# pmgbergen/porepy

Hardware: NVIDIA H100
Metric: 3D cells/sec MPFA+MPSA assembly (higher is better)
Workload: dtype f64

## Files before the change

porepy_b200/csrc/api.cu:

```cuda
#include <cuda_runtime.h>

#include <omp.h>

#include <atomic>
#include <chrono>
#include <thread>
#include <climits>
#include <cstdio>
#include <cstdlib>
#include <cstring>
#include <string>
#include <vector>

#include "plan.hpp"
#include <nvtx3/nvToolsExt.h>

struct NvtxRange {
    explicit NvtxRange(const char *name) { nvtxRangePushA(name); }
    ~NvtxRange() { nvtxRangePop(); }
};

static thread_local std::string g_err;
static thread_local int64_t g_err_node = -1;
static std::atomic<int64_t> g_launches{0};
// ... 27 lines not shown
void pb_set_error_node_(int64_t node) { g_err_node = node; }
extern "C" int64_t pb_launch_count(void) { return g_launches.load(); }
extern "C" int pb_device_count(void) {
    int n = 0;
    if (cudaGetDeviceCount(&n) != cudaSuccess) return -1;
    return n;
}
extern "C" int pb_set_device(int device) {
    CUDA_TRY(cudaSetDevice(device));
    return PB_OK;
}

extern "C" int pb_host_alloc(uint64_t bytes, void **out) {
    if (!out) return fail(PB_EINVAL, "null pointer");
    CUDA_TRY(cudaHostAlloc(out, bytes ? bytes : 8, cudaHostAllocDefault));
    return PB_OK;
}
extern "C" void pb_host_free(void *p) {
    if (p) cudaFreeHost(p);
}

static int64_t cfg_scratch(int cfg, int n) {
    switch (cfg) {
        case 0: return Cfg0::scratch_doubles_c();
        case 1: return Cfg1::scratch_doubles_c();
        case 2: return Cfg2::scratch_doubles_c();
        case 3: return Cfg3::scratch_doubles_c();
        case 4: return Cfg4::scratch_doubles_c();
        case 5: return Cfg5::scratch_doubles_c();
        default: return n;
    }
}

template <class F>
static int build_classes(pb_plan *p, std::vector<NodeClass> &out, F size_of) {
    const HostPlan &H = p->H;
    std::vector<int32_t> lists[2 * kNumCfg];
    int64_t amax[2 * kNumCfg] = {0}, rmax[2 * kNumCfg] = {0}, smax[2 * kNumCfg] = {0};
    for (int64_t s = 0; s < H.nn; ++s) {
        int nsc = H.node_sc_ptr[s + 1] - H.node_sc_ptr[s];
        int nsf = H.node_sf_ptr[s + 1] - H.node_sf_ptr[s];
        if (nsf == 0) continue;
        if (!p->active.empty() && !p->active[s]) continue;
        int n = 0, w = 0;
        int64_t a = 0, r = 0;
        size_of(nsf, nsc, H.node_nb[s], &n, &w, &a, &r);
        int cfg = 0;
        while (cfg < kCatchAll && (n > kCfg[cfg].max_n || w > kCfg[cfg].max_w)) ++cfg;
        const int64_t scr = cfg_scratch(cfg, n);
        const int tpb = kCfg[cfg].team == 32 ? 4 : 1;
        bool glob = (size_t)(a + r + scr) * 8 * tpb > kMaxSmem;
        if (glob && (size_t)(r + scr) * 8 * tpb > kMaxSmem)
            return fail(PB_ENOTIMPL, "interaction region at node " + std::to_string(s) +
                                         " is too large for this build (" + std::to_string(nsf) +
                                         " sub-faces)");
        int key = cfg * 2 + (glob ? 1 : 0);
        lists[key].push_back((int32_t)s);
        amax[key] = std::max(amax[key], a);
        rmax[key] = std::max(rmax[key], r);
        smax[key] = std::max(smax[key], scr);
    }
    out.clear();
    for (int key = 0; key < 2 * kNumCfg; ++key) {
        if (lists[key].empty()) continue;
        out.emplace_back();
        NodeClass &c = out.back();
        c.cfg = key / 2;
        c.a_global = key & 1;
        c.team = kCfg[c.cfg].team;
        c.n = (int)lists[key].size();
        c.a_doubles = amax[key];
        c.rest_doubles = rmax[key];
        c.scr_doubles = smax[key];
        if (!c.a_global) {
            const int tpb = c.team == 32 ? 4 : 1;
            if ((size_t)(c.a_doubles + c.rest_doubles + c.scr_doubles) * 8 * tpb > kMaxSmem) c.a_global = true;
        }
        if (!p->node_key.empty()) {
            const std::vector<uint32_t> &nk = p->node_key;
            std::stable_sort(lists[key].begin(), lists[key].end(), [&](int32_t x, int32_t y) { return nk[x] < nk[y]; });
        }
        if (c.nodes.upload(lists[key], p->stream) != cudaSuccess) return fail(PB_ECUDA, "upload of node list failed");
    }
    return PB_OK;
}

static int build_mpfa_classes(pb_plan *p) {
    const int nd = p->H.nd;
    return build_classes(p, p->mpfa_cls, [&](int nsf, int nsc, int nb, int *n, int *w, int64_t *a, int64_t *r) {
        *n = nsf;
        *w = mpfa_width(nd, nsf, nsc, nb);
        *a = mpfa_A_doubles(nd, nsf, nsc, nb);
        *r = mpfa_rest_doubles(nd, nsf, nsc, nb);
    });
}

template <int CAP>
__global__ void pattern_kernel(int64_t nrows, const int32_t *__restrict__ rn_ptr, const int32_t *__restrict__ rn,
                               const int32_t *__restrict__ col_ptr, const int32_t *__restrict__ col_idx,
                               int32_t *__restrict__ counts, const int32_t *__restrict__ indptr,
                               int32_t *__restrict__ indices, int pass, int *overflow) {
    __shared__ int32_t sbuf[8][CAP];
    const int lane = threadIdx.x & 31, wib = threadIdx.x >> 5;
    int32_t *buf = sbuf[wib];
    const int64_t warp = (int64_t)blockIdx.x * (blockDim.x >> 5) + wib;
    const int64_t nwarps = (int64_t)gridDim.x * (blockDim.x >> 5);
    for (int64_t r = warp; r < nrows; r += nwarps) {
        int total = 0;
        bool over = false;
        for (int q = rn_ptr[r]; q < rn_ptr[r + 1]; ++q) {
            const int s = rn[q];
            const int b = col_ptr[s], len = col_ptr[s + 1] - b;
            if (total + len > CAP) { over = true; break; }
            for (int i = lane; i < len; i += 32) buf[total + i] = col_idx[b + i];
            total += len;
        }
        if (over) {
            if (lane == 0) { atomicExch(overflow, 1); if (pass == 0) counts[r] = 0; }
            continue;
        }
        int P = 1;
        while (P < total) P <<= 1;
// ... 951 lines not shown
    return PB_OK;
}

extern "C" int pb_mpsa_upload(pb_plan *p, const double *stiffness, const uint8_t *bc,
                              const double *robin_weight, double eta, int n_alpha,
                              const double *alpha) {
    NvtxRange nvtx_("pb_mpsa_upload");
    if (!p || !stiffness || !bc) return fail(PB_EINVAL, "null pointer");
    if (!p->have_geo) return fail(PB_EINVAL, "pb_plan_set_geometry has not been called");
    if (n_alpha < 0 || n_alpha > PB_MAX_ALPHA) return fail(PB_EINVAL, "0 <= n_alpha <= 4");
    if (n_alpha > 0 && !alpha) return fail(PB_EINVAL, "null alpha");
    const HostPlan &H = p->H;
    const int nd = H.nd;
    cudaStream_t st = p->stream;
    { int rcs = upload_cell_tensor(p, p->stiff, stiffness, 81); if (rcs) return rcs; }
    CUDA_TRY(p->vbc.upload(bc, (size_t)nd * H.nf, st));
    p->have_vrobw = robin_weight != nullptr;
    p->have_vbasis = false;
    if (robin_weight) CUDA_TRY(p->vrobw.upload(robin_weight, (size_t)nd * nd * H.nf, st));
    if (n_alpha) {
        CUDA_TRY(p->alpha.ensure((size_t)n_alpha * 9 * H.nc * sizeof(double)));
        for (int q = 0; q < n_alpha; ++q) {
            DevBuf one;
            int rca = upload_cell_tensor(p, one, alpha + (size_t)q * 9 * (p->cell_map.p ? p->cell_map_src : H.nc), 9);
            if (rca) return rca;
            CUDA_TRY(cudaMemcpyAsync(p->alpha.as<double>() + (size_t)q * 9 * H.nc, one.p,
                                     (size_t)9 * H.nc * sizeof(double), cudaMemcpyDeviceToDevice, st));
            CUDA_TRY(cudaStreamSynchronize(st));
        }
    }
    p->n_alpha = n_alpha;
    p->veta = eta;
    if (p->mpsa_cls_nalpha != n_alpha) {
        int rc = build_classes(p, p->mpsa_cls, [&](int nsf, int nsc, int nb, int *n, int *w, int64_t *a,
                                                   int64_t *r) {
            *n = nsf * nd;
            *w = mpsa_width(nd, nsf, nsc, nb, n_alpha);
            *a = mpsa_A_doubles(nd, nsf, nsc, nb, n_alpha);
            *r = mpsa_rest_doubles(nd, nsf, nsc, nb, n_alpha);
        });
        if (rc) return rc;
        p->mpsa_cls_nalpha = n_alpha;
    }
    CUDA_TRY(cudaStreamSynchronize(st));
    p->mpsa_ready = true;
    return PB_OK;
}

extern "C" int pb_mpsa_set_basis(pb_plan *p, const double *basis) {
    if (!p) return fail(PB_EINVAL, "null plan");
    if (!p->mpsa_ready) return fail(PB_EINVAL, "pb_mpsa_upload has not been called");
    p->have_vbasis = basis != nullptr;
    if (basis) {
        const HostPlan &H = p->H;
        CUDA_TRY(p->vbasis.upload(basis, (size_t)H.nd * H.nd * H.nf, p->stream));
        CUDA_TRY(cudaStreamSynchronize(p->stream));
    }
    return PB_OK;
}

extern "C" int pb_mpsa_assemble(pb_plan *p, float *ms) {
    NvtxRange nvtx_("pb_mpsa_assemble");
    if (!p) return fail(PB_EINVAL, "null plan");
    if (!p->mpsa_ready) return fail(PB_EINVAL, "pb_mpsa_upload has not been called");
    const HostPlan &H = p->H;
    const int nd = H.nd;
    cudaStream_t st = p->stream;
    const size_t nfc = (size_t)p->pat_nnz[0], nfb = (size_t)p->pat_nnz[1], ncc = (size_t)p->pat_nnz[2], ncb = (size_t)p->pat_nnz[3];
// ... 63 lines not shown
```

porepy_b200/csrc/mpsa_node.cuh:

```cuda
#pragma once
#include "node_kernels.cuh"

namespace pb {

PB_HD int mpsa_width(int nd, int nsf, int nsc, int nb, int nalpha) {
    return (nsf * nd + nsc * nd + nb * nd + nalpha * nsc) | 1;
}
PB_HD int64_t mpsa_A_doubles(int nd, int nsf, int nsc, int nb, int nalpha) {
    return (int64_t)nsf * nd * mpsa_width(nd, nsf, nsc, nb, nalpha);
}
PB_HD int64_t mpsa_rest_doubles(int nd, int nsf, int nsc, int nb, int nalpha) {
    const int64_t nd2 = nd * nd, n = (int64_t)nsf * nd;
    const int64_t nrhs = (int64_t)nsc * nd + (int64_t)nb * nd + (int64_t)nalpha * nsc;
    int64_t d = (int64_t)nsc * nd2 * nd2;
    d += (int64_t)nsc * nd2;
    d += nd2 * (n + (int64_t)nsc * nd);
    d += nd2 * nrhs;
    d += nsf;
    d += (int64_t)nsf * nd;
    d += (int64_t)nsc;
    d += (int64_t)nalpha * nsc * nd2 * 2;
    int64_t ints = nsc + 4 * (int64_t)nsf + (int64_t)nsf * nd + n + (int64_t)nsc * nd + 2 * nd;
    return d + (ints + 1) / 2 + 2;
}

template <int ND>
PB_HD int c9(int i, int r) { return 3 * i + r; }

template <int ND>
PB_HD bool sym_mask(int p, int q) {
    if (p == q) return true;
    return (p % (ND + 1) == 0) && (q % (ND + 1) == 0);
}

template <int ND, class Solver, class Team>
PB_HD void mpsa_node(Team &t, const PlanView &P, const GeoView &G, const MpsaParams &prm,
                     const MpsaOut &o, int64_t s, double *A, double *smd, double *scratch, int *err,
                     int64_t s_next = -1) {
    constexpr int ND2 = ND * ND;
    const int sc0 = P.node_sc_ptr[s], nsc = P.node_sc_ptr[s + 1] - sc0;
    const int sf0 = P.node_sf_ptr[s], nsf = P.node_sf_ptr[s + 1] - sf0;
    const int nb = P.node_nb[s];
    if (nsf == 0) return;
    const int nal = prm.n_alpha;
    const int n = nsf * ND;
    const int ncc = nsc * ND;
    const int nbc = nb * ND;
    const int nrhs = ncc + nbc + nal * nsc;
    const int W = (n + nrhs) | 1;
    const int64_t nf = P.nf, nc = P.nc, nn = P.nn;

    double *PS = smd;
    double *E = PS + nsc * ND2 * ND2;
    double *SA = E + nsc * ND2;
    double *SAc = SA + ND2 * n;
    double *Z = SAc + ND2 * ncc;
    double *invmf = Z + ND2 * nrhs;
    double *nrm = invmf + nsf;
    double *volk = nrm + nsf * ND;
    double *NA = volk + nsc;
    double *AE = NA + nal * nsc * ND2;
    int *cell = (int *)(AE + nal * nsc * ND2);
    int *face = cell + nsc;
    int *sides = face + nsf;
    int *bloc = sides + nsf;
    int *bcu = bloc + nsf;
    int *rowidx = bcu + nsf * ND;
    int *slot = rowidx + n;
    int *elim = slot + nsc * ND;
    int *sidesel = elim + 2 * ND;

    for (int k = t.tid(); k < nsc; k += t.size()) cell[k] = P.sc_cell[sc0 + k];
    for (int i = t.tid(); i < nsc * ND; i += t.size()) slot[i] = P.slot_sf[(int64_t)sc0 * ND + i];
    for (int u = t.tid(); u < nsf; u += t.size()) {
        const int64_t f = P.sf_face[sf0 + u];
        face[u] = (int)f;
        sides[u] = (int)P.sf_sides[sf0 + u];
        const int bl = P.sf_bloc[sf0 + u];
        bloc[u] = (bl == 0xFFFF) ? -1 : bl;
        const double im = 1.0 / (double)(P.fn_indptr[f + 1] - P.fn_indptr[f]);
        invmf[u] = im;
#pragma unroll
        for (int i = 0; i < ND; ++i) {
            int code = 0;
            if (bl != 0xFFFF) {
                code = prm.bc[i * nf + f];
                if (code == 0) code = 2;
            }
            bcu[u * ND + i] = code;
            nrm[u * ND + i] = G.fnorm[i * G.face_cs + f * G.face_es] * im;
        }
    }
    for (int x = t.tid(); x < n; x += t.size()) rowidx[x] = x;
    for (int i = t.tid(); i < n * W; i += t.size()) A[i] = 0.0;
    for (int i = t.tid(); i < ND2 * (n + ncc); i += t.size()) SA[i] = 0.0;
    t.sync();

    for (int k = t.tid(); k < nsc; k += t.size()) {
        const int64_t c = cell[k];
        double xc[ND], xs[ND], D[ND][ND], Ei[ND][ND];
#pragma unroll
        for (int i = 0; i < ND; ++i) {
            xc[i] = G.ccent[i * G.cell_cs + c * G.cell_es];
            xs[i] = G.nodes[i * G.node_cs + s * G.node_es];
        }
#pragma unroll
        for (int m = 0; m < ND; ++m) {
            const int u = slot[k * ND + m] >> 1;
            const int64_t f = face[u];
            const double e = (bloc[u] >= 0) ? 0.0 : prm.eta;
#pragma unroll
            for (int i = 0; i < ND; ++i) {
                const double xf = G.fcent[i * G.face_cs + f * G.face_es];
                D[m][i] = xf + e * (xs[i] - xf) - xc[i];
            }
        }
        if (!invert_small<ND>(D, Ei)) flag_singular(err, s);
#pragma unroll
        for (int q = 0; q < ND; ++q)
#pragma unroll
            for (int m = 0; m < ND; ++m) E[k * ND2 + q * ND + m] = Ei[q][m];
        volk[k] = G.cvol[c] / (double)P.sc_ncn[c];
        for (int q = 0; q < nal; ++q) {
            const double *al = prm.alpha + (int64_t)q * prm.alpha_stride;
            double a2[ND][ND];
#pragma unroll
            for (int a = 0; a < ND; ++a)
// ... 66 lines not shown
        for (int u = 0; u < nsf; ++u) {
            cn += bcu[u * ND + i] == 2;
            cr += bcu[u * ND + i] == 3;
        }
        elim[i] = nsc < cn;
        elim[ND + i] = nsc < cr;
    }
    t.sync();

    for (int u = t.tid(); u < nsf; u += t.size()) {
        const int s1 = sides[u] & 0xFFFF, s2 = (sides[u] >> 16) & 0xFFFF;
        int pick = s1;
        if (s2 != 0xFFFF) {
            const double *nu = nrm + u * ND;
            double w1 = 0.0, w2 = 0.0;
            const double *p1 = PS + (s1 / ND) * ND2 * ND2, *p2 = PS + (s2 / ND) * ND2 * ND2;
            for (int i = 0; i < ND; ++i)
                for (int am = 0; am < ND2; ++am) {
                    double a1 = 0.0, a2 = 0.0;
#pragma unroll
                    for (int r = 0; r < ND; ++r) {
                        a1 += nu[r] * p1[(i * ND + r) * ND2 + am];
                        a2 += nu[r] * p2[(i * ND + r) * ND2 + am];
                    }
                    w1 += fabs(a1);
                    w2 += fabs(a2);
                }
            if (w2 < w1) pick = s2;
        }
        sidesel[u] = pick;
    }
    t.sync();

    for (int x = t.tid(); x < n; x += t.size()) {
        const int u = x / ND, i = x - u * ND;
        double *row = A + (int64_t)x * W;
        const int code = bcu[x];
        if (code == 1 && prm.basis == nullptr) {
            row[x] = 1.0;
            row[n + ncc + bloc[u] * ND + i] = 1.0;
            continue;
        }
        const double *nu = nrm + u * ND;
        if (prm.basis != nullptr && bloc[u] >= 0) {
            const int64_t fb = face[u];
            double B[ND][ND];
#pragma unroll
            for (int a = 0; a < ND; ++a)
#pragma unroll
                for (int j = 0; j < ND; ++j) B[a][j] = prm.basis[(int64_t)(a * ND + j) * nf + fb];
            if (code == 1) {
#pragma unroll
                for (int j = 0; j < ND; ++j) row[u * ND + j] = B[i][j];
                row[n + ncc + bloc[u] * ND + i] = 1.0;
            } else {
                const int side = sides[u] & 0xFFFF;
                const int k = side / ND;
                const double sg = (slot[side] & 1) ? -1.0 : 1.0;
                for (int j = 0; j < ND; ++j) {
                    const double wgt = sg * B[i][j];
                    if (wgt == 0.0) continue;
                    const double *ps = PS + (k * ND2 + j * ND) * ND2;
#pragma unroll
                    for (int a = 0; a < ND; ++a) {
                        double csum = 0.0;
#pragma unroll
                        for (int m = 0; m < ND; ++m) {
                            double v = 0.0;
#pragma unroll
                            for (int r = 0; r < ND; ++r) v += nu[r] * ps[(r * ND + a) * ND + m];
                            v *= wgt;
                            row[(slot[k * ND + m] >> 1) * ND + a] += v;
                            csum += v;
                        }
                        row[n + k * ND + a] += csum;
                    }
                    for (int q = 0; q < nal; ++q)
                        row[n + ncc + nbc + q * nsc + k] += wgt * NA[((q * nsc + k) * ND + (side - k * ND)) * ND + j];
                    const int cj = bcu[u * ND + j];
                    if (!((cj == 2 && elim[j]) || (cj == 3 && elim[ND + j]))) {
                        for (int c = 0; c < n; ++c) {
                            double v = 0.0;
#pragma unroll
                            for (int r = 0; r < ND; ++r) v += nu[r] * SA[(j * ND + r) * n + c];
                            row[c] += wgt * v;
                        }
                        for (int c = 0; c < ncc; ++c) {
                            double v = 0.0;
#pragma unroll
                            for (int r = 0; r < ND; ++r) v += nu[r] * SAc[(j * ND + r) * ncc + c];
                            row[n + c] -= wgt * v;
                        }
                    }
                }
                row[n + ncc + bloc[u] * ND + i] = invmf[u];
                if (code == 3) {
                    const double as = G.farea[fb] * invmf[u];
#pragma unroll
                    for (int j = 0; j < ND; ++j) {
                        double wb = 0.0;
#pragma unroll
                        for (int kk = 0; kk < ND; ++kk)
                            wb += (prm.robw ? prm.robw[(int64_t)(i * ND + kk) * nf + fb] : (i == kk ? 1.0 : 0.0)) * B[kk][j];
                        row[u * ND + j] += as * wb;
                    }
                }
            }
            double sum = 0.0;
            for (int c = 0; c < n; ++c) sum += fabs(row[c]);
            if (!(sum > 0.0)) { flag_singular(err, s); continue; }
            const double is = 1.0 / sum;
            for (int c = 0; c < n + nrhs; ++c) row[c] *= is;
            continue;
        }
        for (int sd = 0; sd < 2; ++sd) {
            const int side = sd == 0 ? (sides[u] & 0xFFFF) : ((sides[u] >> 16) & 0xFFFF);
            if (side == 0xFFFF) continue;
            const int k = side / ND;
            const double sg = (slot[side] & 1) ? -1.0 : 1.0;
            const double *ps = PS + (k * ND2 + i * ND) * ND2;
#pragma unroll
            for (int a = 0; a < ND; ++a) {
                double csum = 0.0;
#pragma unroll
                for (int m = 0; m < ND; ++m) {
                    double v = 0.0;
#pragma unroll
                    for (int r = 0; r < ND; ++r) v += nu[r] * ps[(r * ND + a) * ND + m];
                    v *= sg;
                    row[(slot[k * ND + m] >> 1) * ND + a] += v;
                    csum += v;
                }
                row[n + k * ND + a] += csum;
            }
            for (int q = 0; q < nal; ++q)
                row[n + ncc + nbc + q * nsc + k] += sg * NA[((q * nsc + k) * ND + (side - k * ND)) * ND + i];
            if (code != 0) {
                const bool el = code == 2 ? elim[i] : elim[ND + i];
                if (!el) {
                    for (int c = 0; c < n; ++c) {
                        double v = 0.0;
#pragma unroll
                        for (int r = 0; r < ND; ++r) v += nu[r] * SA[(i * ND + r) * n + c];
                        row[c] += sg * v;
                    }
                    for (int c = 0; c < ncc; ++c) {
                        double v = 0.0;
#pragma unroll
                        for (int r = 0; r < ND; ++r) v += nu[r] * SAc[(i * ND + r) * ncc + c];
                        row[n + c] -= sg * v;
                    }
                }
            }
        }
        if (code == 2 || code == 3) row[n + ncc + bloc[u] * ND + i] = invmf[u];
        if (code == 3) {
            const int64_t f = face[u];
            const double as = G.farea[f] * invmf[u];
#pragma unroll
            for (int j = 0; j < ND; ++j) {
                const double w = prm.robw ? prm.robw[(int64_t)(i * ND + j) * nf + f] : (i == j ? 1.0 : 0.0);
                row[u * ND + j] += as * w;
            }
        }
        double sum = 0.0;
        for (int c = 0; c < n; ++c) sum += fabs(row[c]);
        if (!(sum > 0.0)) { flag_singular(err, s); continue; }
        const double is = 1.0 / sum;
        for (int c = 0; c < n + nrhs; ++c) row[c] *= is;
    }
    t.sync();

    if (!Solver::solve(t, A, n, W, nrhs, rowidx, scratch)) {
        if (t.tid() == 0) flag_singular(err, s);
        t.sync();
        return;
    }

#if defined(__CUDA_ARCH__)
    int pf_sc0 = 0, pf_nsc = 0, pf_sf0 = 0, pf_nsf = 0;
    int64_t pf_pos0 = 0;
    if (s_next >= 0) {
        pf_sc0 = P.node_sc_ptr[s_next];
        pf_nsc = P.node_sc_ptr[s_next + 1] - pf_sc0;
        pf_sf0 = P.node_sf_ptr[s_next];
        pf_nsf = P.node_sf_ptr[s_next + 1] - pf_sf0;
        pf_pos0 = P.posfc_ptr[s_next];
    }
#endif
#if defined(__CUDA_ARCH__)
    {
        const int l = t.lane();
        const int ntr = (ND2 + 15) / 16, ntc = (nrhs + 7) / 8;
        for (int tile = t.warp(); tile < ntr * ntc; tile += t.nwarps()) {
            const int tr = tile / ntc, tc = tile - tr * ntc;
            const int row0 = 16 * tr + (l >> 2), row1 = row0 + 8;
            const int colb = 8 * tc + (l >> 2);
            double acc0[2] = {0.0, 0.0}, acc1[2] = {0.0, 0.0};
            for (int k0 = 0; k0 < n; k0 += 4) {
                const int k = k0 + (l & 3);
                const double a0 = (row0 < ND2 && k < n) ? SA[row0 * n + k] : 0.0;
                const double a1 = (row1 < ND2 && k < n) ? SA[row1 * n + k] : 0.0;
                const double b = (k < n && colb < nrhs) ? A[(int64_t)rowidx[k] * W + n + colb] : 0.0;
                pb_dmma2(acc0, acc1, a0, a1, b);
            }
            const int c0 = 8 * tc + 2 * (l & 3);
            const int rows[2] = {row0, row1};
            const double *accs[2] = {acc0, acc1};
            for (int h = 0; h < 2; ++h) {
                const int row = rows[h];
                if (row < ND2) {
                    if (c0 < nrhs) Z[row * nrhs + c0] = accs[h][0] + (c0 < ncc ? SAc[row * ncc + c0] : 0.0);
                    if (c0 + 1 < nrhs)
                        Z[row * nrhs + c0 + 1] = accs[h][1] + (c0 + 1 < ncc ? SAc[row * ncc + c0 + 1] : 0.0);
                }
            }
        }
    }
#else
    for (int it = t.tid(); it < ND2 * nrhs; it += t.size()) {
        const int p = it / nrhs, c = it - p * nrhs;
        double v = (c < ncc) ? SAc[p * ncc + c] : 0.0;
        for (int x = 0; x < n; ++x) v += SA[p * n + x] * A[(int64_t)rowidx[x] * W + n + c];
        Z[it] = v;
    }
#endif
    t.sync();

#if defined(__CUDA_ARCH__)
    int pf_cell = -1, pf_face = -1;
    if (t.tid() < pf_nsc) pf_cell = P.sc_cell[pf_sc0 + t.tid()];
    if (t.tid() < pf_nsf) {
        pf_face = P.sf_face[pf_sf0 + t.tid()];
        if ((t.tid() & 7) == 0) {
            pb_prefetch_l2(P.sf_sides + pf_sf0 + t.tid());
            pb_prefetch_l2(P.sf_bloc + pf_sf0 + t.tid());
        }
    }
    if (t.tid() * 16 < pf_nsc * ND) pb_prefetch_l2(P.slot_sf + (int64_t)pf_sc0 * ND + t.tid() * 16);
    for (int64_t off = (int64_t)t.tid() * 32; off < (int64_t)pf_nsf * pf_nsc; off += (int64_t)t.size() * 32)
        pb_prefetch_l2(P.pos_fc + pf_pos0 + off);
#endif
    const int32_t *pfc = P.pos_fc + P.posfc_ptr[s];
    const int32_t *pfb = P.pos_fb + P.posfb_ptr[s];
    for (int u = t.warp(); u < nsf; u += t.nwarps()) {
        const double *nu = nrm + u * ND;
        const int side1 = sidesel[u];
        const int k1 = side1 / ND, m1 = side1 - k1 * ND;
        double hs[ND][ND][ND];
        double hsum[ND][ND];
#pragma unroll
        for (int i = 0; i < ND; ++i) {
            const double *ps1 = PS + (k1 * ND2 + i * ND) * ND2;
#pragma unroll
            for (int a = 0; a < ND; ++a) {
                double sm = 0.0;
#pragma unroll
                for (int m = 0; m < ND; ++m) {
                    double v = 0.0;
#pragma unroll
                    for (int r = 0; r < ND; ++r) v += nu[r] * ps1[(r * ND + a) * ND + m];
                    hs[i][a][m] = v;
                    sm += v;
                }
                hsum[i][a] = sm;
            }
        }
        int xo[ND][ND];
#pragma unroll
        for (int a = 0; a < ND; ++a)
#pragma unroll
            for (int m = 0; m < ND; ++m) xo[a][m] = rowidx[(slot[k1 * ND + m] >> 1) * ND + a] * W + n;
        bool use_asym[ND];
        int uo[ND];
#pragma unroll
        for (int i = 0; i < ND; ++i) {
            const int code = bcu[u * ND + i];
            use_asym[i] = !((code == 2 && elim[i]) || (code == 3 && elim[ND + i]));
            uo[i] = rowidx[u * ND + i] * W + n;
        }
        const double im = invmf[u];
        const int64_t f = face[u];
        const int64_t fc0 = P.fc_indptr[f], fcl = P.fc_indptr[f + 1] - fc0;
        const int64_t fb0 = P.fb_indptr[f], fbl = P.fb_indptr[f + 1] - fb0;
        for (int c = t.lane(); c < nrhs; c += t.lanes()) {
            double hk[ND], tr[ND];
#pragma unroll
            for (int i = 0; i < ND; ++i) hk[i] = 0.0;
#pragma unroll
            for (int a = 0; a < ND; ++a)
#pragma unroll
                for (int m = 0; m < ND; ++m) {
                    const double xv = A[xo[a][m] + c];
#pragma unroll
                    for (int i = 0; i < ND; ++i) hk[i] += hs[i][a][m] * xv;
                }
#pragma unroll
            for (int i = 0; i < ND; ++i) {
                if (use_asym[i]) {
#pragma unroll
                    for (int r = 0; r < ND; ++r) hk[i] += nu[r] * Z[(i * ND + r) * nrhs + c];
                }
                tr[i] = A[uo[i] + c] * im;
            }
            if (c < ncc) {
                const int k = c / ND, j = c - k * ND;
                if (k == k1) {
#pragma unroll
                    for (int i = 0; i < ND; ++i) {
                        double hj = hsum[i][0];
#pragma unroll
                        for (int a = 1; a < ND; ++a) hj = (j == a) ? hsum[i][a] : hj;
                        hk[i] -= hj;
                    }
                }
                const int64_t pb = pfc[u * nsc + k];
                const int64_t pos = ND2 * fc0 + (pb - fc0) * ND + j;
#pragma unroll
                for (int i = 0; i < ND; ++i) {
                    if (o.stress) red_add(o.stress + pos + (int64_t)i * ND * fcl, hk[i]);
                    if (o.bdc) red_add(o.bdc + pos + (int64_t)i * ND * fcl, tr[i]);
                }
            } else if (c < ncc + nbc) {
                const int cb = c - ncc;
                const int b = cb / ND, j = cb - b * ND;
                const int64_t pb = pfb[u * nb + b];
                const int64_t pos = ND2 * fb0 + (pb - fb0) * ND + j;
#pragma unroll
                for (int i = 0; i < ND; ++i) {
                    if (o.bstress) red_add(o.bstress + pos + (int64_t)i * ND * fbl, hk[i]);
                    if (o.bdf) red_add(o.bdf + pos + (int64_t)i * ND * fbl, tr[i]);
                }
            } else {
                const int cq = c - ncc - nbc;
                const int q = cq / nsc, k = cq - q * nsc;
                const int64_t pb = pfc[u * nsc + k];
// ... 13 lines not shown
        if (prm.stiff_cs == 1) {
            const double *rec = prm.stiff + (int64_t)pf_cell * prm.stiff_es;
#pragma unroll
            for (int b = 0; b < 81; b += 16) pb_prefetch_l2(rec + b);
            pb_prefetch_l2(rec + 80);
        }
        if (G.cell_cs == 1) pb_prefetch_l2(G.ccent + (int64_t)pf_cell * G.cell_es);
        pb_prefetch_l2(G.cvol + pf_cell);
        pb_prefetch_l2(P.sc_ncn + pf_cell);
    }
    if (pf_face >= 0) {
        if (G.face_cs == 1) {
            pb_prefetch_l2(G.fnorm + (int64_t)pf_face * G.face_es);
            pb_prefetch_l2(G.fcent + (int64_t)pf_face * G.face_es);
        }
        pb_prefetch_l2(P.fn_indptr + pf_face);
        pb_prefetch_l2(P.fc_indptr + pf_face);
#pragma unroll
        for (int i = 0; i < ND; ++i) pb_prefetch_l2(prm.bc + (int64_t)i * nf + pf_face);
    }
#endif
    if (nal > 0) {
        const int32_t *pcc = P.pos_cc + P.poscc_ptr[s];
        const int32_t *pcb = P.pos_cb + P.poscb_ptr[s];
        for (int it = t.warp(); it < nal * nsc; it += t.nwarps()) {
            const int q = it / nsc, k = it - q * nsc;
            const double *ae = AE + (q * nsc + k) * ND2;
            const double vol = volk[k];
            const double *xr[ND][ND];
#pragma unroll
            for (int a = 0; a < ND; ++a)
#pragma unroll
                for (int m = 0; m < ND; ++m)
                    xr[a][m] = A + (int64_t)rowidx[(slot[k * ND + m] >> 1) * ND + a] * W + n;
            for (int c = t.lane(); c < nrhs; c += t.lanes()) {
                double v = 0.0;
#pragma unroll
                for (int a = 0; a < ND; ++a)
#pragma unroll
                    for (int m = 0; m < ND; ++m) v += ae[a * ND + m] * xr[a][m][c];
                if (c < ncc) {
                    const int k2 = c / ND, j = c - k2 * ND;
                    if (k2 == k) {
#pragma unroll
                        for (int m = 0; m < ND; ++m) v -= ae[j * ND + m];
                    }
                    if (o.dd[q]) red_add(o.dd[q] + (int64_t)pcc[k * nsc + k2] * ND + j, vol * v);
                } else if (c < ncc + nbc) {
                    const int cb = c - ncc;
                    const int b = cb / ND, j = cb - b * ND;
                    if (o.bdd[q]) red_add(o.bdd[q] + (int64_t)pcb[k * nb + b] * ND + j, vol * v);
                } else {
                    const int cq = c - ncc - nbc;
                    const int q2 = cq / nsc, k2 = cq - q2 * nsc;
                    if (q2 == q && o.cons[q]) red_add(o.cons[q] + (int64_t)pcc[k * nsc + k2], vol * v);
                }
            }
        }
    }
    t.sync();
}

}
```

porepy_b200/csrc/node_kernels.cuh:

```cuda
#pragma once
#include <cmath>
#include <cstdint>

#include "views.hpp"

namespace pb {

struct CpuTeam {
    PB_HD int tid() const { return 0; }
    PB_HD int size() const { return 1; }
    PB_HD int lanes() const { return 1; }
    PB_HD int warp() const { return 0; }
    PB_HD int nwarps() const { return 1; }
    PB_HD int lane() const { return 0; }
    PB_HD void sync() const {}
    PB_HD void warp_argmax(double &, int &) const {}
};

#if defined(__CUDACC__)
template <int TEAM>
struct GpuTeam {
    __device__ __forceinline__ int tid() const { return TEAM == 32 ? (threadIdx.x & 31) : threadIdx.x; }
    __device__ __forceinline__ int size() const { return TEAM; }
    __device__ __forceinline__ int lanes() const { return 32; }
// ... 51 lines not shown
            }
            t.warp_argmax(best, bi);
            if (t.lane() == 0) {
                int r = rowidx[bi];
                rowidx[bi] = rowidx[p];
                rowidx[p] = r;
                ipiv[p] = (best > 0.0) ? 1.0 / A[r * W + p] : 0.0;
            }
        }
        t.sync();
        const int pr = rowidx[p];
        const double inv = ipiv[p];
        if (inv == 0.0 || !(inv == inv)) ok = false;
        const int c0 = p + 1;
        const int wend = n + nrhs;
        for (int li = t.warp(); li < n; li += t.nwarps()) {
            if (li == p) continue;
            const int ri = rowidx[li];
            const double f = A[ri * W + p] * inv;
            if (f == 0.0) continue;
            for (int c = c0 + t.lane(); c < wend; c += t.lanes()) A[ri * W + c] -= f * A[pr * W + c];
        }
        t.sync();
    }
    for (int p = t.warp(); p < n; p += t.nwarps()) {
        const int pr = rowidx[p];
        const double inv = ipiv[p];
        for (int c = n + t.lane(); c < n + nrhs; c += t.lanes()) A[pr * W + c] *= inv;
    }
    t.sync();
    return ok;
}

struct SmemGJ {
    static constexpr int team = 256;
    static constexpr int min_blocks = 1;
    static PB_HD int64_t scratch_doubles(int n) { return n; }
    template <class Team>
    static PB_HD bool solve(Team &t, double *A, int n, int W, int nrhs, int *rowidx, double *scratch) {
        return gauss_jordan(t, A, n, W, nrhs, rowidx, scratch);
    }
};

#if defined(__CUDACC__)
__device__ __forceinline__ void pb_dmma(double (&c)[2], double a, double b) {
    asm volatile("mma.sync.aligned.m8n8k4.row.col.f64.f64.f64.f64 {%0,%1}, {%2}, {%3}, {%0,%1};"
                 : "+d"(c[0]), "+d"(c[1])
                 : "d"(a), "d"(b));
}
__device__ __forceinline__ void pb_dmma2(double (&c0)[2], double (&c1)[2], double a0, double a1, double b) {
    asm volatile("mma.sync.aligned.m16n8k4.row.col.f64.f64.f64.f64 {%0,%1,%2,%3}, {%4,%5}, {%6}, {%0,%1,%2,%3};"
                 : "+d"(c0[0]), "+d"(c0[1]), "+d"(c1[0]), "+d"(c1[1])
                 : "d"(a0), "d"(a1), "d"(b));
}

template <int NW, int RT, int NCT, int MINB>
struct TileGJ {
    static_assert(NCT % 2 == 0, "padded row stride must be 4 mod 16");
    static constexpr int team = NW * 32;
    static constexpr int min_blocks = MINB;
    static constexpr int NRT = NW * RT;
    static constexpr int max_n = NRT * 8;
    static constexpr int max_w = NCT * 8;
    static constexpr int NP = ((max_n + 31) / 32) * 32;
    static constexpr int NI = NP / 32;
    static constexpr int WP = NCT * 8 + 4;
    static_assert(NP <= 256, "row index must fit the 8-bit key field");
    static_assert(NI <= 8, "extend the PB_PICK list");
    static __host__ __device__ constexpr int64_t scratch_doubles_c() {
        return NP * 4 + 2 * 4 * WP + 16 * (NW + 1) + (8 + NP) / 2 + 4;
    }
    static PB_HD int64_t scratch_doubles(int) { return scratch_doubles_c(); }

// ... 95 lines not shown
                    const double rpiv = __drcp_rn(prow[j]);
#pragma unroll
                    for (int i = 0; i < NI; ++i) {
                        const bool me = (l == ol) && (i == os);
                        if (me) us[i] = true;
                        else {
                            const double f = v[i][j] * rpiv;
#pragma unroll
                            for (int jj = j + 1; jj < 4; ++jj) v[i][jj] -= f * prow[jj];
                        }
                    }
                }
            }
        }
        int prj = -1;
#pragma unroll
        for (int j = 0; j < 4; ++j)
            if (j == mj) prj = mypr[j];
        const double m = (prj >= 0) ? ((mi < pw) ? P0[prj * 4 + mi] : 0.0) : (mi == mj ? 1.0 : 0.0);
        const double growth = invert_block(l, m, iv);
        if (!(growth < 1e300)) sing = true;
        if (l < 16) Ainv[l] = iv;
        if (l == 0) {
#pragma unroll
            for (int j = 0; j < 4; ++j) {
                prs[j] = mypr[j];
                if (mypr[j] >= 0) { usedf[mypr[j]] = 1; rowidx[p0 + j] = mypr[j]; }
            }
            if (sing) prs[4] = 1;
        }
    }


    template <class Team>
    static __device__ __forceinline__ bool solve(Team &t, double *A, int n, int W, int nrhs,
                                                 int *rowidx, double *scratch) {
        const int ti = t.warp(), l = t.lane();
        const int gr = l >> 2, gc = (l & 3) * 2;
        const int wend = n + nrhs;
        double c[RT][NCT][2];
#pragma unroll
        for (int rt = 0; rt < RT; ++rt) {
            const int myrow = 8 * (ti + NW * rt) + gr;
#pragma unroll
            for (int tc = 0; tc < NCT; ++tc) {
                const int col = 8 * tc + gc;
                c[rt][tc][0] = (myrow < n && col < wend) ? A[myrow * W + col] : 0.0;
                c[rt][tc][1] = (myrow < n && col + 1 < wend) ? A[myrow * W + col + 1] : 0.0;
            }
        }
        double *P0 = scratch;
        double *Raw = P0 + NP * 4;
        double *R = Raw + 4 * WP;
        double *Ainv = R + 4 * WP;
        int *prs = (int *)(Ainv + 16 * (NW + 1));
        int *usedf = prs + 8;
        for (int i = t.tid(); i < NP; i += t.size()) usedf[i] = i < n ? 0 : 1;
        for (int i = t.tid(); i < NP * 4; i += t.size()) P0[i] = 0.0;
        if (t.tid() == 0) prs[4] = 0;
        t.sync();
        const int npanel = (n + 3) >> 2;
        bool ok = true;
#pragma unroll
        for (int tcp = 0; tcp < NRT && tcp < NCT; ++tcp) {
            for (int half = 0; half < 2; ++half) {
                const int q = 2 * tcp + half;
                if (q >= npanel || !ok) break;
                const int p0 = 4 * q;
                const int pw = (n - p0) < 4 ? (n - p0) : 4;
                if (((l & 3) >> 1) == half) {
                    const int j0 = 2 * (l & 1);
#pragma unroll
                    for (int rt = 0; rt < RT; ++rt) {
                        const int myrow = 8 * (ti + NW * rt) + gr;
                        P0[myrow * 4 + j0] = c[rt][tcp][0];
                        P0[myrow * 4 + j0 + 1] = c[rt][tcp][1];
                    }
                }
                int myp[RT];
#pragma unroll
                for (int rt = 0; rt < RT; ++rt) {
                    const int myrow = 8 * (ti + NW * rt) + gr;
                    const int j = myrow - p0;
// ... 56 lines not shown
                    rowidx[p0 + t.tid()] = p0 + t.tid();
                }
                {
                    const int k = l & 3;
                    const int src = (l & ~3) | (2 * half + (k >> 1));
                    double af[RT];
#pragma unroll
                    for (int rt = 0; rt < RT; ++rt) {
                        const double v0 = __shfl_sync(0xffffffffu, c[rt][tcp][0], src);
                        const double v1 = __shfl_sync(0xffffffffu, c[rt][tcp][1], src);
                        af[rt] = (k < pw) ? -((k & 1) ? v1 : v0) : 0.0;
                    }
                    const double *rb = R + k * WP + (l >> 2);
#pragma unroll
                    for (int tc = tcp; tc < NCT; ++tc) {
                        const double bf = rb[8 * tc];
#pragma unroll
                        for (int rt = 0; rt + 1 < RT; rt += 2) pb_dmma2(c[rt][tc], c[rt + 1][tc], af[rt], af[rt + 1], bf);
                        if (RT & 1) pb_dmma(c[RT - 1][tc], af[RT - 1], bf);
                    }
#pragma unroll
                    for (int rt = 0; rt < RT; ++rt)
                        if (myp[rt] >= 0) {
#pragma unroll
                            for (int tc = tcp; tc < NCT; ++tc) {
                                c[rt][tc][0] = R[myp[rt] * WP + 8 * tc + gc];
                                c[rt][tc][1] = R[myp[rt] * WP + 8 * tc + gc + 1];
                            }
                        }
                }
            }
        }
        t.sync();
        if (!ok) return false;
#pragma unroll
        for (int rt = 0; rt < RT; ++rt) {
            const int myrow = 8 * (ti + NW * rt) + gr;
#pragma unroll
            for (int tc = 0; tc < NCT; ++tc) {
                const int col = 8 * tc + gc;
                if (myrow < n) {
                    if (col >= n && col < wend) A[myrow * W + col] = c[rt][tc][0];
                    if (col + 1 >= n && col + 1 < wend) A[myrow * W + col + 1] = c[rt][tc][1];
                }
            }
        }
        t.sync();
        return true;
    }
};
#endif

#if defined(__CUDACC__)
__device__ __forceinline__ void pb_prefetch_l2(const void *p) {
    asm volatile("prefetch.global.L2 [%0];" ::"l"(p));
}
#endif

template <int ND>
PB_HD bool invert_small(const double (&D)[ND][ND], double (&E)[ND][ND]);

template <>
PB_HD bool invert_small<2>(const double (&D)[2][2], double (&E)[2][2]) {
    double det = D[0][0] * D[1][1] - D[0][1] * D[1][0];
    if (det == 0.0 || !(det == det)) return false;
    double id = 1.0 / det;
    E[0][0] = D[1][1] * id; E[0][1] = -D[0][1] * id;
    E[1][0] = -D[1][0] * id; E[1][1] = D[0][0] * id;
    return true;
}

template <>
PB_HD bool invert_small<3>(const double (&D)[3][3], double (&E)[3][3]) {
    double c00 = D[1][1] * D[2][2] - D[1][2] * D[2][1];
    double c01 = D[1][2] * D[2][0] - D[1][0] * D[2][2];
    double c02 = D[1][0] * D[2][1] - D[1][1] * D[2][0];
    double det = D[0][0] * c00 + D[0][1] * c01 + D[0][2] * c02;
    if (det == 0.0 || !(det == det)) return false;
    double id = 1.0 / det;
    E[0][0] = c00 * id;
    E[1][0] = c01 * id;
// ... 207 lines not shown
```

porepy_b200/csrc/plan.hpp:

```cpp
#pragma once
#include <cuda_runtime.h>

#include <algorithm>
#include <atomic>
#include <chrono>
#include <climits>
#include <cstdint>
#include <cstdio>
#include <cstdlib>
#include <cstring>
#include <map>
#include <mutex>
#include <string>
#include <vector>

#include "../../include/poreb200.h"
#include "mpsa_node.cuh"
#include "face_kernels.cuh"
#include "node_kernels.cuh"
#include "plan_host.hpp"

int pb_fail_(int code, const std::string &msg);
void pb_count_launch_();
void pb_set_error_node_(int64_t node);
// ... 162 lines not shown
    static int cache[64] = {0};
    int dev = 0;
    if (cudaGetDevice(&dev) != cudaSuccess || dev < 0 || dev >= 64) dev = 0;
    if (!cache[dev]) {
        int n = 0;
        if (cudaDeviceGetAttribute(&n, cudaDevAttrMultiProcessorCount, dev) != cudaSuccess || n < 1) n = 1;
        cache[dev] = n;
    }
    return cache[dev];
}


#define PB_LAUNCH_CFG(KERNEL, ND, ...)                                              \
    switch (c.cfg) {                                                                \
        case 0: rc = launch_one(KERNEL<ND, Cfg0>, c, p, __VA_ARGS__); break;        \
        case 1: rc = launch_one(KERNEL<ND, Cfg1>, c, p, __VA_ARGS__); break;        \
        case 2: rc = launch_one(KERNEL<ND, Cfg2>, c, p, __VA_ARGS__); break;        \
        case 3: rc = launch_one(KERNEL<ND, Cfg3>, c, p, __VA_ARGS__); break;        \
        case 4: rc = launch_one(KERNEL<ND, Cfg4>, c, p, __VA_ARGS__); break;        \
        case 5: rc = launch_one(KERNEL<ND, Cfg5>, c, p, __VA_ARGS__); break;        \
        default: rc = launch_one(KERNEL<ND, Cfg6>, c, p, __VA_ARGS__); break;       \
    }

template <class K, class Prm, class Out>
static int launch_one(K kernel, const NodeClass &c, pb_plan *p, const Prm &prm, const Out &o) {
    const int blk = c.team == 32 ? 128 : c.team;
    const int tpb = blk / c.team;
    const size_t smem = (size_t)(c.scr_doubles + c.rest_doubles + (c.a_global ? 0 : c.a_doubles)) *
                        sizeof(double) * tpb;
    if (smem > kMaxSmem)
        return pb_fail_(PB_ENOTIMPL, "interaction region needs " + std::to_string(smem) +
                                     " B of shared memory (> 227 KB)");
    CUDA_TRY(cudaFuncSetAttribute(kernel, cudaFuncAttributeMaxDynamicSharedMemorySize, (int)smem));
    int per_sm = 1;
    CUDA_TRY(cudaOccupancyMaxActiveBlocksPerMultiprocessor(&per_sm, kernel, blk, smem));
    if (per_sm < 1) per_sm = 1;
    int64_t need = ((int64_t)c.n + tpb - 1) / tpb;
    int grid = (int)std::max<int64_t>(1, std::min<int64_t>(need, (int64_t)pb_sm_count() * per_sm));
    double *ws = nullptr;
    if (c.a_global) {
        CUDA_TRY(p->a_ws.ensure((size_t)grid * tpb * c.a_doubles * sizeof(double)));
        ws = p->a_ws.as<double>();
    }
    kernel<<<grid, blk, smem, p->stream>>>(p->view, p->geo, prm, o, c.nodes.as<int32_t>(), c.n,
                                           (int)c.scr_doubles, (int)c.rest_doubles,
                                           (int)c.a_doubles, ws, p->err.as<int>());
    pb_count_launch_();
    CUDA_TRY(cudaGetLastError());
    return PB_OK;
}


int pb_launch_mpfa_(pb_plan *p, const MpfaParams &prm, const MpfaOut &o);
int pb_launch_mpsa2_(pb_plan *p, const MpsaParams &prm, const MpsaOut &o);
int pb_launch_mpsa3_(pb_plan *p, const MpsaParams &prm, const MpsaOut &o);
int pb_upload_repacked_(cudaStream_t st, DevBuf &tmp, DevBuf &dst, const double *host, int ncomp, int64_t n);
int pb_build_device_topology_(pb_plan *p, int nd, int64_t nc, int64_t nf, int64_t nn, const int32_t *cf_indptr,
                              const int32_t *cf_indices, const int8_t *cf_data, const int32_t *fn_indptr,
                              const int32_t *fn_indices, DevBuf &fn_idx_dev, std::string &err);
```

Before: 6.840 million.

## Fill MPSA rows directly into solver register tiles and shrink smem pool

MPSA assembly no longer builds the full n×W augmented matrix in shared memory. It passes a row-fill callback to the solver, which fills 8-row tiles per warp into a small buffer, normalises them and loads them straight into the elimination registers. The solution is then written to a compact padded X array. This reduces the per-node shared-memory footprint, which can raise occupancy or keep more nodes off the global-A path. A separate change sets the shared-memory carveout preference from the computed need, which may leave more L1 cache available.

```diff
diff --git a/porepy_b200/csrc/api.cu b/porepy_b200/csrc/api.cu
--- a/porepy_b200/csrc/api.cu
+++ b/porepy_b200/csrc/api.cu
@@ -83,8 +83,20 @@
     }
 }
 
+static int64_t cfg_pool(int cfg, int n, int w) {
+    switch (cfg) {
+        case 0: return Cfg0::pool_doubles(n, w);
+        case 1: return Cfg1::pool_doubles(n, w);
+        case 2: return Cfg2::pool_doubles(n, w);
+        case 3: return Cfg3::pool_doubles(n, w);
+        case 4: return Cfg4::pool_doubles(n, w);
+        case 5: return Cfg5::pool_doubles(n, w);
+        default: return Cfg6::pool_doubles(n, w);
+    }
+}
+
 template <class F>
-static int build_classes(pb_plan *p, std::vector<NodeClass> &out, F size_of) {
+static int build_classes(pb_plan *p, std::vector<NodeClass> &out, bool rows_to_solver, F size_of) {
     const HostPlan &H = p->H;
     std::vector<int32_t> lists[2 * kNumCfg];
     int64_t amax[2 * kNumCfg] = {0}, rmax[2 * kNumCfg] = {0}, smax[2 * kNumCfg] = {0};
@@ -107,7 +119,7 @@
                                          " sub-faces)");
         int key = cfg * 2 + (glob ? 1 : 0);
         lists[key].push_back((int32_t)s);
-        amax[key] = std::max(amax[key], a);
+        amax[key] = std::max(amax[key], rows_to_solver ? cfg_pool(cfg, n, w) : a);
         rmax[key] = std::max(rmax[key], r);
         smax[key] = std::max(smax[key], scr);
     }
@@ -138,7 +150,7 @@
 
 static int build_mpfa_classes(pb_plan *p) {
     const int nd = p->H.nd;
-    return build_classes(p, p->mpfa_cls, [&](int nsf, int nsc, int nb, int *n, int *w, int64_t *a, int64_t *r) {
+    return build_classes(p, p->mpfa_cls, false, [&](int nsf, int nsc, int nb, int *n, int *w, int64_t *a, int64_t *r) {
         *n = nsf;
         *w = mpfa_width(nd, nsf, nsc, nb);
         *a = mpfa_A_doubles(nd, nsf, nsc, nb);
@@ -1156,8 +1168,8 @@
     p->n_alpha = n_alpha;
     p->veta = eta;
     if (p->mpsa_cls_nalpha != n_alpha) {
-        int rc = build_classes(p, p->mpsa_cls, [&](int nsf, int nsc, int nb, int *n, int *w, int64_t *a,
-                                                   int64_t *r) {
+        int rc = build_classes(p, p->mpsa_cls, true, [&](int nsf, int nsc, int nb, int *n, int *w, int64_t *a,
+                                                         int64_t *r) {
             *n = nsf * nd;
             *w = mpsa_width(nd, nsf, nsc, nb, n_alpha);
             *a = mpsa_A_doubles(nd, nsf, nsc, nb, n_alpha);
diff --git a/porepy_b200/csrc/mpsa_node.cuh b/porepy_b200/csrc/mpsa_node.cuh
--- a/porepy_b200/csrc/mpsa_node.cuh
+++ b/porepy_b200/csrc/mpsa_node.cuh
@@ -35,7 +35,7 @@
 
 template <int ND, class Solver, class Team>
 PB_HD void mpsa_node(Team &t, const PlanView &P, const GeoView &G, const MpsaParams &prm,
-                     const MpsaOut &o, int64_t s, double *A, double *smd, double *scratch, int *err,
+                     const MpsaOut &o, int64_t s, double *pool, double *smd, double *scratch, int *err,
                      int64_t s_next = -1) {
     constexpr int ND2 = ND * ND;
     const int sc0 = P.node_sc_ptr[s], nsc = P.node_sc_ptr[s + 1] - sc0;
@@ -47,7 +47,6 @@
     const int ncc = nsc * ND;
     const int nbc = nb * ND;
     const int nrhs = ncc + nbc + nal * nsc;
-    const int W = (n + nrhs) | 1;
     const int64_t nf = P.nf, nc = P.nc, nn = P.nn;
 
     double *PS = smd;
@@ -92,7 +91,6 @@
         }
     }
     for (int x = t.tid(); x < n; x += t.size()) rowidx[x] = x;
-    for (int i = t.tid(); i < n * W; i += t.size()) A[i] = 0.0;
     for (int i = t.tid(); i < ND2 * (n + ncc); i += t.size()) SA[i] = 0.0;
     t.sync();
 
@@ -225,14 +223,13 @@
     }
     t.sync();
 
-    for (int x = t.tid(); x < n; x += t.size()) {
+    auto row_of = [&](int x, double *row) {
         const int u = x / ND, i = x - u * ND;
-        double *row = A + (int64_t)x * W;
         const int code = bcu[x];
         if (code == 1 && prm.basis == nullptr) {
             row[x] = 1.0;
             row[n + ncc + bloc[u] * ND + i] = 1.0;
-            continue;
+            return;
         }
         const double *nu = nrm + u * ND;
         if (prm.basis != nullptr && bloc[u] >= 0) {
@@ -299,12 +296,7 @@
                     }
                 }
             }
-            double sum = 0.0;
-            for (int c = 0; c < n; ++c) sum += fabs(row[c]);
-            if (!(sum > 0.0)) { flag_singular(err, s); continue; }
-            const double is = 1.0 / sum;
-            for (int c = 0; c < n + nrhs; ++c) row[c] *= is;
-            continue;
+            return;
         }
         for (int sd = 0; sd < 2; ++sd) {
             const int side = sd == 0 ? (sides[u] & 0xFFFF) : ((sides[u] >> 16) & 0xFFFF);
@@ -356,15 +348,11 @@
                 row[u * ND + j] += as * w;
             }
         }
-        double sum = 0.0;
-        for (int c = 0; c < n; ++c) sum += fabs(row[c]);
-        if (!(sum > 0.0)) { flag_singular(err, s); continue; }
-        const double is = 1.0 / sum;
-        for (int c = 0; c < n + nrhs; ++c) row[c] *= is;
-    }
-    t.sync();
-
-    if (!Solver::solve(t, A, n, W, nrhs, rowidx, scratch)) {
+    };
+
+    const double *X;
+    int ldx;
+    if (!Solver::solve_rows(t, row_of, n, nrhs, pool, rowidx, scratch, X, ldx)) {
         if (t.tid() == 0) flag_singular(err, s);
         t.sync();
         return;
@@ -394,7 +382,7 @@
                 const int k = k0 + (l & 3);
                 const double a0 = (row0 < ND2 && k < n) ? SA[row0 * n + k] : 0.0;
                 const double a1 = (row1 < ND2 && k < n) ? SA[row1 * n + k] : 0.0;
-                const double b = (k < n && colb < nrhs) ? A[(int64_t)rowidx[k] * W + n + colb] : 0.0;
+                const double b = (k < n && colb < nrhs) ? X[rowidx[k] * ldx + colb] : 0.0;
                 pb_dmma2(acc0, acc1, a0, a1, b);
             }
             const int c0 = 8 * tc + 2 * (l & 3);
@@ -414,7 +402,7 @@
     for (int it = t.tid(); it < ND2 * nrhs; it += t.size()) {
         const int p = it / nrhs, c = it - p * nrhs;
         double v = (c < ncc) ? SAc[p * ncc + c] : 0.0;
-        for (int x = 0; x < n; ++x) v += SA[p * n + x] * A[(int64_t)rowidx[x] * W + n + c];
+        for (int x = 0; x < n; ++x) v += SA[p * n + x] * X[(int64_t)rowidx[x] * ldx + c];
         Z[it] = v;
     }
 #endif
@@ -463,14 +451,14 @@
 #pragma unroll
         for (int a = 0; a < ND; ++a)
 #pragma unroll
-            for (int m = 0; m < ND; ++m) xo[a][m] = rowidx[(slot[k1 * ND + m] >> 1) * ND + a] * W + n;
+            for (int m = 0; m < ND; ++m) xo[a][m] = rowidx[(slot[k1 * ND + m] >> 1) * ND + a] * ldx;
         bool use_asym[ND];
         int uo[ND];
 #pragma unroll
         for (int i = 0; i < ND; ++i) {
             const int code = bcu[u * ND + i];
             use_asym[i] = !((code == 2 && elim[i]) || (code == 3 && elim[ND + i]));
-            uo[i] = rowidx[u * ND + i] * W + n;
+            uo[i] = rowidx[u * ND + i] * ldx;
         }
         const double im = invmf[u];
         const int64_t f = face[u];
@@ -484,7 +472,7 @@
             for (int a = 0; a < ND; ++a)
 #pragma unroll
                 for (int m = 0; m < ND; ++m) {
-                    const double xv = A[xo[a][m] + c];
+                    const double xv = X[xo[a][m] + c];
 #pragma unroll
                     for (int i = 0; i < ND; ++i) hk[i] += hs[i][a][m] * xv;
                 }
@@ -494,7 +482,7 @@
 #pragma unroll
                     for (int r = 0; r < ND; ++r) hk[i] += nu[r] * Z[(i * ND + r) * nrhs + c];
                 }
-                tr[i] = A[uo[i] + c] * im;
+                tr[i] = X[uo[i] + c] * im;
             }
             if (c < ncc) {
                 const int k = c / ND, j = c - k * ND;
@@ -574,7 +562,7 @@
             for (int a = 0; a < ND; ++a)
 #pragma unroll
                 for (int m = 0; m < ND; ++m)
-                    xr[a][m] = A + (int64_t)rowidx[(slot[k * ND + m] >> 1) * ND + a] * W + n;
+                    xr[a][m] = X + (int64_t)rowidx[(slot[k * ND + m] >> 1) * ND + a] * ldx;
             for (int c = t.lane(); c < nrhs; c += t.lanes()) {
                 double v = 0.0;
 #pragma unroll
diff --git a/porepy_b200/csrc/node_kernels.cuh b/porepy_b200/csrc/node_kernels.cuh
--- a/porepy_b200/csrc/node_kernels.cuh
+++ b/porepy_b200/csrc/node_kernels.cuh
@@ -107,13 +107,40 @@
     return ok;
 }
 
+template <class Team, class Fill>
+PB_HD void fill_system(Team &t, const Fill &fill, int n, int nrhs, double *A, int W) {
+    for (int i = t.tid(); i < n * W; i += t.size()) A[i] = 0.0;
+    t.sync();
+    for (int x = t.tid(); x < n; x += t.size()) {
+        double *row = A + (int64_t)x * W;
+        fill(x, row);
+        double sum = 0.0;
+        for (int c = 0; c < n; ++c) sum += fabs(row[c]);
+        if (sum > 0.0) {
+            const double is = 1.0 / sum;
+            for (int c = 0; c < n + nrhs; ++c) row[c] *= is;
+        }
+    }
+    t.sync();
+}
+
 struct SmemGJ {
     static constexpr int team = 256;
     static constexpr int min_blocks = 1;
     static PB_HD int64_t scratch_doubles(int n) { return n; }
+    static PB_HD int64_t pool_doubles(int n, int W) { return (int64_t)n * W; }
     template <class Team>
     static PB_HD bool solve(Team &t, double *A, int n, int W, int nrhs, int *rowidx, double *scratch) {
         return gauss_jordan(t, A, n, W, nrhs, rowidx, scratch);
+    }
+    template <class Team, class Fill>
+    static PB_HD bool solve_rows(Team &t, const Fill &fill, int n, int nrhs, double *pool, int *rowidx,
+                                 double *scratch, const double *&X, int &ldx) {
+        const int W = (n + nrhs) | 1;
+        fill_system(t, fill, n, nrhs, pool, W);
+        X = pool + n;
+        ldx = W;
+        return gauss_jordan(t, pool, n, W, nrhs, rowidx, scratch);
     }
 };
 
@@ -275,6 +302,14 @@
     }
 
 
+    static PB_HD int x_stride(int nrhs) { return ((nrhs + 11) / 16) * 16 + 4; }
+    static constexpr bool kFillTiles = NW > 2;
+    static PB_HD int64_t pool_doubles(int n, int W) {
+        if (!kFillTiles) return (int64_t)n * W;
+        const int64_t x = (int64_t)n * x_stride(W - n), f = (int64_t)NW * 8 * W;
+        return x > f ? x : f;
+    }
+
     template <class Team>
     static __device__ __forceinline__ bool solve(Team &t, double *A, int n, int W, int nrhs,
                                                  int *rowidx, double *scratch) {
@@ -292,6 +327,90 @@
                 c[rt][tc][1] = (myrow < n && col + 1 < wend) ? A[myrow * W + col + 1] : 0.0;
             }
         }
+        if (!eliminate(t, c, n, rowidx, scratch)) return false;
+        store(t, c, n, nrhs, A + n, W);
+        return true;
+    }
+
+    template <class Team, class Fill>
+    static __device__ __forceinline__ bool solve_rows(Team &t, const Fill &fill, int n, int nrhs, double *pool,
+                                                      int *rowidx, double *scratch, const double *&X, int &ldx) {
+        const int ti = t.warp(), l = t.lane();
+        const int gr = l >> 2, gc = (l & 3) * 2;
+        const int wend = n + nrhs;
+        const int W = wend | 1;
+        if constexpr (!kFillTiles) {
+            fill_system(t, fill, n, nrhs, pool, W);
+            X = pool + n;
+            ldx = W;
+            return solve(t, pool, n, W, nrhs, rowidx, scratch);
+        }
+        double *buf = pool + (int64_t)ti * 8 * W;
+        double c[RT][NCT][2];
+#pragma unroll
+        for (int rt = 0; rt < RT; ++rt)
+#pragma unroll
+            for (int tc = 0; tc < NCT; ++tc) c[rt][tc][0] = c[rt][tc][1] = 0.0;
+#pragma unroll 1
+        for (int ps = 0; ps < RT; ++ps) {
+            const int r0 = 8 * (ti + NW * ps);
+            if (r0 >= n) break;
+            for (int i = l; i < 8 * W; i += 32) buf[i] = 0.0;
+            __syncwarp();
+            if (l < 8 && r0 + l < n) fill(r0 + l, buf + l * W);
+            __syncwarp();
+            const double *row = buf + gr * W;
+            double sum = 0.0;
+            for (int cc = l & 3; cc < n; cc += 4) sum += fabs(row[cc]);
+            sum += __shfl_xor_sync(0xffffffffu, sum, 1);
+            sum += __shfl_xor_sync(0xffffffffu, sum, 2);
+            const double is = sum > 0.0 ? 1.0 / sum : 1.0;
+            const int myrow = r0 + gr;
+#pragma unroll
+            for (int rt = 0; rt < RT; ++rt) {
+                if (rt == ps && myrow < n) {
+#pragma unroll
+                    for (int tc = 0; tc < NCT; ++tc) {
+                        const int col = 8 * tc + gc;
+                        if (col < wend) c[rt][tc][0] = row[col] * is;
+                        if (col + 1 < wend) c[rt][tc][1] = row[col + 1] * is;
+                    }
+                }
+            }
+            __syncwarp();
+        }
+        if (!eliminate(t, c, n, rowidx, scratch)) return false;
+        ldx = x_stride(nrhs);
+        store(t, c, n, nrhs, pool, ldx);
+        X = pool;
+        return true;
+    }
+
+    template <class Team>
+    static __device__ __forceinline__ void store(Team &t, const double (&c)[RT][NCT][2], int n, int nrhs,
+                                                 double *X, int ldx) {
+        const int ti = t.warp(), l = t.lane();
+        const int gr = l >> 2, gc = (l & 3) * 2;
+#pragma unroll
+        for (int rt = 0; rt < RT; ++rt) {
+            const int myrow = 8 * (ti + NW * rt) + gr;
+#pragma unroll
+            for (int tc = 0; tc < NCT; ++tc) {
+                const int col = 8 * tc + gc - n;
+                if (myrow < n) {
+                    if (col >= 0 && col < nrhs) X[myrow * ldx + col] = c[rt][tc][0];
+                    if (col + 1 >= 0 && col + 1 < nrhs) X[myrow * ldx + col + 1] = c[rt][tc][1];
+                }
+            }
+        }
+        t.sync();
+    }
+
+    template <class Team>
+    static __device__ __forceinline__ bool eliminate(Team &t, double (&c)[RT][NCT][2], int n, int *rowidx,
+                                                     double *scratch) {
+        const int ti = t.warp(), l = t.lane();
+        const int gr = l >> 2, gc = (l & 3) * 2;
         double *P0 = scratch;
         double *Raw = P0 + NP * 4;
         double *R = Raw + 4 * WP;
@@ -414,21 +533,7 @@
             }
         }
         t.sync();
-        if (!ok) return false;
-#pragma unroll
-        for (int rt = 0; rt < RT; ++rt) {
-            const int myrow = 8 * (ti + NW * rt) + gr;
-#pragma unroll
-            for (int tc = 0; tc < NCT; ++tc) {
-                const int col = 8 * tc + gc;
-                if (myrow < n) {
-                    if (col >= n && col < wend) A[myrow * W + col] = c[rt][tc][0];
-                    if (col + 1 >= n && col + 1 < wend) A[myrow * W + col + 1] = c[rt][tc][1];
-                }
-            }
-        }
-        t.sync();
-        return true;
+        return ok;
     }
 };
 #endif
diff --git a/porepy_b200/csrc/plan.hpp b/porepy_b200/csrc/plan.hpp
--- a/porepy_b200/csrc/plan.hpp
+++ b/porepy_b200/csrc/plan.hpp
@@ -218,9 +218,18 @@
         return pb_fail_(PB_ENOTIMPL, "interaction region needs " + std::to_string(smem) +
                                      " B of shared memory (> 227 KB)");
     CUDA_TRY(cudaFuncSetAttribute(kernel, cudaFuncAttributeMaxDynamicSharedMemorySize, (int)smem));
+    CUDA_TRY(cudaFuncSetAttribute(kernel, cudaFuncAttributePreferredSharedMemoryCarveout, cudaSharedmemCarveoutDefault));
     int per_sm = 1;
     CUDA_TRY(cudaOccupancyMaxActiveBlocksPerMultiprocessor(&per_sm, kernel, blk, smem));
     if (per_sm < 1) per_sm = 1;
+    {
+        static const int kCarveKB[] = {0, 8, 16, 32, 64, 100, 132, 164, 196, 228};
+        const size_t need = (smem + 1024) * (size_t)per_sm;
+        int pct = 100;
+        for (int kb : kCarveKB)
+            if ((size_t)kb * 1024 >= need) { pct = kb * 100 / 228; break; }
+        CUDA_TRY(cudaFuncSetAttribute(kernel, cudaFuncAttributePreferredSharedMemoryCarveout, pct));
+    }
     int64_t need = ((int64_t)c.n + tpb - 1) / tpb;
     int grid = (int)std::max<int64_t>(1, std::min<int64_t>(need, (int64_t)pb_sm_count() * per_sm));
     double *ws = nullptr;
```

Measured after the change: 7.331 million, median of 6. +7.2%, better.
